# ishine/zerovox.cpp

Measured on AMD Instinct MI355X. Metric: audio-seconds/wall-second (xRT) end-to-end phoneme->22.05 kHz wav, higher is better.
Workload: dtype f16*f16->f32 (MFMA) convs, f32 (MFMA) attention/linear, f32 activations

## Files before the change

zerovox.cpp_amd/csrc/conv1d_mfma.hip:

```cpp
#include "kernels.h"
#include "knobs.h"
#include "mfma_common.h"
#include "tile_deal.h"

#include <hip/hip_fp16.h>
#include <algorithm>
#include <cstdlib>
#include <cstring>

namespace zv
{

#ifndef ZV_ST_AUX
#define ZV_ST_AUX 2
#endif
#ifdef ZV_ABL_A
#define ZV_ABL_LD(arr, p, mt) ((mt) == 0 ? *(const half8 *)(p) : arr[0])
#else
#define ZV_ABL_LD(arr, p, mt) (*(const half8 *)((p) + (mt) * 32 * RS))
#endif
#ifndef ZV_STAGE_U128
#define ZV_STAGE_U128 12
#endif
#ifndef ZV_STAGE_U256
// ... 94 lines not shown

void pack_pair_weight(const uint16_t *w, int K, int C, int Cp, uint16_t *dst)
{
    const int nkc = Cp / 16;
    const size_t seg = (size_t)(round_up(K * nkc, 4) + 8) * 512;
    memset(dst, 0, pair_weight_halfs(Cp, K) * 2);
    for (int nt = 0; nt < Cp / 32; nt++)
        for (int tap = 0; tap < K; tap++)
            for (int kc = 0; kc < nkc; kc++)
            {
                uint16_t *d = dst + nt * seg + (size_t)(tap * nkc + kc) * 512;
                for (int lane = 0; lane < 64; lane++)
                    for (int j = 0; j < 8; j++)
                    {
                        const int oc = nt * 32 + (lane & 31), ic = kc * 16 + 8 * (lane >> 5) + j;
                        d[lane * 8 + j] = (oc < C && ic < C) ? w[((size_t)oc * C + ic) * K + tap] : (uint16_t)0;
                    }
            }
}

__device__ __forceinline__ float lrelu_max(float x, float s)
{
    float r;
    const float xs = x * s;
    asm("v_max_f32 %0, %1, %2" : "=v"(r) : "v"(x), "v"(xs));
    return r;
}

__device__ __forceinline__ float lrelu_max_pre(float x, float xs)
{
    float r;
    asm("v_max_f32 %0, %1, %2" : "=v"(r) : "v"(x), "v"(xs));
    return r;
}

typedef unsigned int u32x4 __attribute__((ext_vector_type(4)));

typedef _Float16 half2v __attribute__((ext_vector_type(2)));

__device__ __forceinline__ uint2 lrelu4_f16(float x0, float x1, float x2, float x3, float sl)
{
    const float2v a = {x0, x1}, c = {x2, x3};
    const float2v as = a * sl, cs = c * sl;
    const float2v ra = {lrelu_max_pre(a[0], as[0]), lrelu_max_pre(a[1], as[1])};
    const float2v rc = {lrelu_max_pre(c[0], cs[0]), lrelu_max_pre(c[1], cs[1])};
    const half2v ha = __builtin_convertvector(ra, half2v), hc = __builtin_convertvector(rc, half2v);
    uint2 pk;
    pk.x = *(const unsigned int *)&ha;
    pk.y = *(const unsigned int *)&hc;
    return pk;
}


template <int U, int CP>
__device__ __forceinline__ void stage_act_buf(__amdgpu_buffer_rsrc_t rsrc, char *smem, int row_t0, int rows, int tid, float slope)
{
    constexpr int RS = CP * 2 + 16, COLS = CP / 4, SH = (CP == 32) ? 3 : (CP == 64 ? 4 : (CP == 128 ? 5 : 6));
    const int total = rows * COLS;
    for (int base = tid; base < total; base += 256 * U)
    {
        u32x4 v[U];
#pragma unroll
        for (int u = 0; u < U; u++)
        {
            const int idx = base + u * 256;
            const int r = idx >> SH, c4 = idx & (COLS - 1);
            const int voff = (idx < total) ? ((row_t0 + r) * CP + c4 * 4) * 4 : -16;
            v[u] = __builtin_amdgcn_raw_buffer_load_b128(rsrc, voff, 0, 0);
        }
#pragma unroll
        for (int u = 0; u < U; u++)
        {
            const int idx = base + u * 256;
            if (idx < total)
            {
                const int r = idx >> SH, c4 = idx & (COLS - 1);
                half4 h;
                h[0] = (_Float16)lrelu_max(__uint_as_float(v[u].x), slope);
                h[1] = (_Float16)lrelu_max(__uint_as_float(v[u].y), slope);
                h[2] = (_Float16)lrelu_max(__uint_as_float(v[u].z), slope);
                h[3] = (_Float16)lrelu_max(__uint_as_float(v[u].w), slope);
                *(half4 *)(smem + r * RS + c4 * 8) = h;
            }
        }
    }
}


size_t pair_weight16_halfs(int Cp, int K) { return pair_weight_halfs(Cp, K); }

void pack_pair_weight16(const uint16_t *w, int K, int C, int Cp, uint16_t *dst, bool conv2_layout)
{
    const int nk2 = Cp / 32;
    const size_t seg = (size_t)(round_up(K * (Cp / 16), 4) + 8) * 512;
    memset(dst, 0, pair_weight16_halfs(Cp, K) * 2);
    for (int nt = 0; nt < Cp / 32; nt++)
        for (int tap = 0; tap < K; tap++)
            for (int k2 = 0; k2 < nk2; k2++)
                for (int wt = 0; wt < 2; wt++)
                {
                    uint16_t *d = dst + nt * seg + ((size_t)(tap * nk2 + k2) * 2 + wt) * 512;
                    for (int lane = 0; lane < 64; lane++)
                        for (int j = 0; j < 8; j++)
                        {
                            const int r = lane & 15, g = lane >> 4;
                            const int oc = nt * 32 + (conv2_layout ? 2 * r + wt : 16 * wt + r), ic = k2 * 32 + 8 * g + j;
                            d[lane * 8 + j] = (oc < C && ic < C) ? w[((size_t)oc * C + ic) * K + tap] : (uint16_t)0;
                        }
                }
}

template <int MT, int NT, bool SWAP, bool ZERO = false>
__device__ __forceinline__ void mfma16_step(floatx4 (&acc)[MT][NT][2][2], const half8 (&l)[MT][2], const half8 (&w)[NT][2])
{
    const floatx4 z = {0.f, 0.f, 0.f, 0.f};
#pragma unroll
    for (int mt = 0; mt < MT; mt++)
#pragma unroll
        for (int nt = 0; nt < NT; nt++)
#pragma unroll
            for (int wt = 0; wt < 2; wt++)
#pragma unroll
                for (int lt = 0; lt < 2; lt++)
                {
                    if constexpr (SWAP)
                        acc[mt][nt][wt][lt] = __builtin_amdgcn_mfma_f32_16x16x32_f16(w[nt][wt], l[mt][lt], ZERO ? z : acc[mt][nt][wt][lt], 0, 0, 0);
                    else
                        acc[mt][nt][wt][lt] = __builtin_amdgcn_mfma_f32_16x16x32_f16(l[mt][lt], w[nt][wt], ZERO ? z : acc[mt][nt][wt][lt], 0, 0, 0);
                }
}

template <int NT>
__device__ __forceinline__ void deep16_preload_b(half8 (&b0)[2][NT][2], const half8 *wq, size_t wseg)
{
#pragma unroll
    for (int u = 0; u < 2; u++)
#pragma unroll
        for (int nt = 0; nt < NT; nt++)
#pragma unroll
            for (int wt = 0; wt < 2; wt++) b0[u][nt][wt] = wq[nt * wseg + (u * 2 + wt) * 64];
}

template <int CP, int MT, int NT, bool SWAP>
__device__ __forceinline__ void mfma16_taps_deep(floatx4 (&acc)[MT][NT][2][2], const char *ap, int dilRS, const half8 *wq, size_t wseg, int K,
                                                 half8 (&b0)[2][NT][2])
{
    constexpr int RS = CP * 2 + 16, NK2 = CP / 32;
    constexpr int TPB = (NK2 >= 4) ? 1 : 4 / NK2;
    constexpr bool HALF = NK2 == 8;
    const int nsb = (K * NK2 + 1) >> 1;
    const int nb = nsb >> 1;
    half8 b1[2][NT][2];
    wq += 4 * 64;
    half8 a[4][MT][2];
#define ZV16_UN(un) ((un) >= 4 ? (un) - 4 : 0)
#define ZV16_A_ADDR(un) ((un) >= 4 ? tbn[(ZV16_UN(un) / NK2) % 4] + (ZV16_UN(un) % NK2) * 64 : tb[((un) / NK2) % 4] + ((un) % NK2) * 64)
#define ZV16_LOAD_A(un)                                                                                          \
    {                                                                                                            \
        const char *np_ = ZV16_A_ADDR(un);                                                                       \
        _Pragma("unroll") for (int mt = 0; mt < MT; mt++)                                                        \
            _Pragma("unroll") for (int lt = 0; lt < 2; lt++) a[(un) % 4][mt][lt] = *(const half8 *)(np_ + (mt * 32 + lt) * RS); \
    }
#define ZV16_STEP(u, bset) ZV16_LOAD_A((u) + 1) mfma16_step<MT, NT, SWAP>(acc, a[(u) % 4], bset[(u) % 2]); __builtin_amdgcn_sched_barrier(0);
#define ZV16_STEPZ(u, bset) ZV16_LOAD_A((u) + 1) mfma16_step<MT, NT, SWAP, true>(acc, a[(u) % 4], bset[(u) % 2]); __builtin_amdgcn_sched_barrier(0);
#define ZV16_BODY(FIRSTSTEP)                                                                                     \
    {                                                                                                            \
// ... 211 lines not shown
}
#endif

size_t pair_ring_weight_halfs(int Cp, int K) { return (size_t)K * (Cp / 16) * (Cp / 32) * 512; }

void pack_pair_weight_ring(const uint16_t *w, int K, int C, int Cp, uint16_t *dst, bool conv2_layout)
{
    const int nk2 = Cp / 32, nnt = Cp / 32;
    for (int tap = 0; tap < K; tap++)
        for (int k2 = 0; k2 < nk2; k2++)
            for (int nt = 0; nt < nnt; nt++)
                for (int wt = 0; wt < 2; wt++)
                {
                    uint16_t *d = dst + ((((size_t)(tap * nk2 + k2) * nnt + nt) * 2) + wt) * 512;
                    for (int lane = 0; lane < 64; lane++)
                        for (int j = 0; j < 8; j++)
                        {
                            const int r = lane & 15, g = lane >> 4;
                            const int oc = nt * 32 + (conv2_layout ? 2 * r + wt : 16 * wt + r), ic = k2 * 32 + 8 * g + j;
                            d[lane * 8 + j] = (oc < C && ic < C) ? w[((size_t)oc * C + ic) * K + tap] : (uint16_t)0;
                        }
                }
}

template <bool MERGE>
__global__ __launch_bounds__(256, 2) void resblock_pair64_kernel(const PairJobs jobs)
{
    constexpr int CP = 64, MT = 2, NT = 2, BM = 256, RS = CP * 2 + 16;
    constexpr int CHUNK = 8 * 1024;
    const int jz = (int)blockIdx.z, bx = (int)blockIdx.x;
    const int TM = BM - (MERGE ? jobs.kmax - 1 : jobs.j[jz].K - 1);
    const int tps = (jobs.segs.max_rows * jobs.rate + TM - 1) / TM;
    const int vt = tile_deal(bx, tps, jobs.segs.nseg, jobs.deal_c);
    if (vt >= tps * jobs.segs.nseg) return;
    const int useg = vt / tps;
    const Seg sg = seg_at(jobs.segs, useg);
    const int L = sg.rows * jobs.rate;
    const int t0 = (vt - useg * tps) * TM;
    if (t0 >= L) return;

#ifdef ZV_STAMPS
    const int stamp_wg = (int)(blockIdx.x + gridDim.x * blockIdx.z);
    if (jobs.stamp && threadIdx.x == 0 && stamp_wg < ZV_STAMP_WGS)
    {
        jobs.stamp[(size_t)stamp_wg * ZV_STAMP_N + 8] = __builtin_amdgcn_s_getreg(63492);
        jobs.stamp[(size_t)stamp_wg * ZV_STAMP_N + 9] = __builtin_amdgcn_s_getreg(63508);
    }
#endif
    ZV_STAMP(0)
    extern __shared__ __attribute__((aligned(1024))) char smem[];
    char *ring = smem + jobs.ring_off;
    const int tid = threadIdx.x;
    const int lane = tid & 63;
    const int wave = __builtin_amdgcn_readfirstlane(tid >> 6);
    const int lc = lane & 15, lg = lane >> 4;
    const char *abase = smem + (wave * 32 * MT + 2 * lc) * RS + lg * 16;
    const char *bl = ring + lane * 16;

    floatx4 msum[MERGE ? MT : 1][MERGE ? NT : 1][2][2];
    for (int jb = MERGE ? 0 : jz; jb < (MERGE ? jobs.njobs : jz + 1); jb++)
    {
        const PairJob &P = jobs.j[jb];
        const int K = P.K, dil = P.dil;
        const int h2 = (K - 1) / 2, h1 = h2 * dil;
        const float *y_seg = P.y + (size_t)sg.row0 * jobs.rate * CP;
        float *out_seg = (MERGE ? jobs.merge_out : P.out) + (size_t)sg.row0 * jobs.rate * CP;
        const int nchunk = 2 * K;
        const uint64_t w1a = (uint64_t)P.w1r + wave * 2048, w2a = (uint64_t)P.w2r + wave * 2048 - (uint64_t)K * CHUNK;
        const uint32_t w1lo = __builtin_amdgcn_readfirstlane((uint32_t)w1a), w1hi = __builtin_amdgcn_readfirstlane((uint32_t)(w1a >> 32));
        const uint32_t w2lo = __builtin_amdgcn_readfirstlane((uint32_t)w2a), w2hi = __builtin_amdgcn_readfirstlane((uint32_t)(w2a >> 32));
        auto issue = [&](int g) {
            const uint64_t base = g < K ? ((uint64_t)w1hi << 32 | w1lo) : ((uint64_t)w2hi << 32 | w2lo);
            const char *src = (const char *)base + (size_t)g * CHUNK + lane * 16;
            char *dst = ring + (g & 3) * CHUNK + wave * 2048;
            __builtin_amdgcn_global_load_lds((const __attribute__((address_space(1))) void *)src, (__attribute__((address_space(3))) void *)dst, 16, 0, 0);
            __builtin_amdgcn_global_load_lds((const __attribute__((address_space(1))) void *)(src + 1024), (__attribute__((address_space(3))) void *)(dst + 1024), 16, 0, 0);
        };
        if (MERGE && jb) __syncthreads();
        issue(0);
        issue(1);
        issue(2);

        const __amdgpu_buffer_rsrc_t rs_y = __builtin_amdgcn_make_buffer_rsrc((void *)y_seg, 0, L * CP * 4, 0x00020000);
        stage_act_buf<20, CP>(rs_y, smem, t0 - h2 - h1, BM + 2 * h1 + dil, tid, P.slope);
        const int nrows = (L - t0 < TM) ? (L - t0) : TM;
        const __amdgpu_buffer_rsrc_t rs_res = __builtin_amdgcn_make_buffer_rsrc((void *)(y_seg + (size_t)t0 * CP), 0, nrows * CP * 4, 0x00020000);
        const int voff0 = ((wave * 32 * MT + 8 * lg) * CP + 2 * lc) * 4;
        typedef unsigned int u32x2 __attribute__((ext_vector_type(2)));
        u32x2 resv[MT][NT][2][4];
        auto load_res = [&]() {
#pragma unroll
            for (int nt = 0; nt < NT; nt++)
#pragma unroll
                for (int mt = 0; mt < MT; mt++)
#pragma unroll
                    for (int lt = 0; lt < 2; lt++)
#pragma unroll
                        for (int i = 0; i < 4; i++)
                            resv[mt][nt][lt][i] = __builtin_amdgcn_raw_buffer_load_b64(rs_res, voff0 + nt * 128, (mt * 32 + 2 * i + lt) * CP * 4, 0);
        };
        if constexpr (!MERGE) load_res();
        ZV_STAMP(1)
        __syncthreads();
        ZV_STAMP(2)

        floatx4 acc[MT][NT][2][2];
        half8 a[2][MT][2], b[2][NT][2];
        int g = 0;
#define ZV_LDR(slot, aptr, boff)                                                                                      \
    {                                                                                                                 \
        const char *ap_ = (aptr);                                                                                     \
        _Pragma("unroll") for (int mt = 0; mt < MT; mt++)                                                             \
            _Pragma("unroll") for (int lt = 0; lt < 2; lt++) a[slot][mt][lt] = *(const half8 *)(ap_ + (mt * 32 + lt) * RS);    \
        _Pragma("unroll") for (int nt = 0; nt < NT; nt++)                                                             \
            _Pragma("unroll") for (int wt = 0; wt < 2; wt++) b[slot][nt][wt] = *(const half8 *)(bp_ + (boff) + (nt * 2 + wt) * 1024); \
    }
#define ZV_MF(slot, SW, Z)                                \
    mfma16_step<MT, NT, SW, Z>(acc, a[slot], b[slot]);    \
    __builtin_amdgcn_sched_barrier(0);
#define ZV_TAP(SW, Z0, tapstride)                                                                         \
    {                                                                                                     \
        const char *bp_ = bl + (g & 3) * CHUNK, *bn_ = bl + ((g + 1) & 3) * CHUNK;                        \
        ZV_LDR(1, ap + 64, 4 * 1024) ZV_MF(0, SW, Z0)                                                     \
        if (g + 2 < nchunk) asm volatile("s_waitcnt vmcnt(2)" ::: "memory");                              \
        else asm volatile("s_waitcnt vmcnt(0)" ::: "memory");                                             \
        __builtin_amdgcn_s_barrier();                                                                     \
        if (g + 3 < nchunk) issue(g + 3);                                                                 \
        __builtin_amdgcn_sched_barrier(0);                                                                \
        ap += (tapstride);                                                                                \
        bp_ = bn_;                                                                                        \
        ZV_LDR(0, ap, 0) ZV_MF(1, SW, false)                                                              \
        g++;                                                                                              \
    }
        {
            const char *ap = abase;
            {
                const char *bp_ = bl;
                ZV_LDR(0, ap, 0)
            }
            ZV_TAP(true, true, dil * RS)
            for (int tap = 1; tap < K; tap++) ZV_TAP(true, false, dil * RS)
        }
        ZV_STAMP(3)
        asm volatile("s_waitcnt lgkmcnt(0)" ::: "memory");
        __builtin_amdgcn_s_barrier();

        ZV_STAMP(4)
        {
            const float sl = P.slope;
            const bool edge = t0 - h2 < 0 || t0 - h2 + BM > L;
#pragma unroll
            for (int nt = 0; nt < NT; nt++)
            {
                float4 bq[2];
#pragma unroll
                for (int wt = 0; wt < 2; wt++) bq[wt] = *(const float4 *)(P.b1 + nt * 32 + 16 * wt + 4 * lg);
#pragma unroll
                for (int mt = 0; mt < MT; mt++)
#pragma unroll
                    for (int lt = 0; lt < 2; lt++)
                    {
                        const int i = wave * 32 * MT + mt * 32 + 2 * lc + lt;
                        const int t = t0 - h2 + i;
                        const bool in = !edge || (t >= 0 && t < L);
#pragma unroll
                        for (int wt = 0; wt < 2; wt++)
                        {
                            uint2 pk = lrelu4_f16(acc[mt][nt][wt][lt][0] + bq[wt].x, acc[mt][nt][wt][lt][1] + bq[wt].y,
                                                  acc[mt][nt][wt][lt][2] + bq[wt].z, acc[mt][nt][wt][lt][3] + bq[wt].w, sl);
                            if (edge)
                            {
                                pk.x = in ? pk.x : 0u;
                                pk.y = in ? pk.y : 0u;
                            }
                            *(uint2 *)(smem + i * RS + (nt * 32 + 16 * wt + 4 * lg) * 2) = pk;
                        }
                    }
            }
        }
        asm volatile("s_waitcnt lgkmcnt(0)" ::: "memory");
        __builtin_amdgcn_s_barrier();

        ZV_STAMP(5)
        {
            const char *ap = abase;
            {
                const char *bp_ = bl + (g & 3) * CHUNK;
                ZV_LDR(0, ap, 0)
            }
            ZV_TAP(false, true, RS)
            for (int tap = 1; tap < K; tap++) ZV_TAP(false, false, RS)
        }
#undef ZV_TAP
#undef ZV_MF
#undef ZV_LDR

        ZV_STAMP(6)
        if constexpr (MERGE) load_res();
        const __amdgpu_buffer_rsrc_t rs_out = __builtin_amdgcn_make_buffer_rsrc((void *)(out_seg + (size_t)t0 * CP), 0, nrows * CP * 4, 0x00020000);
#pragma unroll
        for (int nt = 0; nt < NT; nt++)
        {
            const float2 bias = *(const float2 *)(P.b2 + nt * 32 + 2 * lc);
            const int voff = voff0 + nt * 128;
#pragma unroll
            for (int mt = 0; mt < MT; mt++)
#pragma unroll
                for (int lt = 0; lt < 2; lt++)
#pragma unroll
                    for (int i = 0; i < 4; i++)
                    {
                        float v0 = (acc[mt][nt][0][lt][i] + bias.x) + __uint_as_float(resv[mt][nt][lt][i][0]);
                        float v1 = (acc[mt][nt][1][lt][i] + bias.y) + __uint_as_float(resv[mt][nt][lt][i][1]);
                        if constexpr (MERGE)
                        {
                            msum[mt][nt][0][lt][i] = jb == 0 ? v0 : msum[mt][nt][0][lt][i] + v0;
                            msum[mt][nt][1][lt][i] = jb == 0 ? v1 : msum[mt][nt][1][lt][i] + v1;
                            if (jb != jobs.njobs - 1) continue;
                            v0 = msum[mt][nt][0][lt][i];
                            v1 = msum[mt][nt][1][lt][i];
                        }
                        const u32x2 o = {__float_as_uint(v0), __float_as_uint(v1)};
                        __builtin_amdgcn_raw_buffer_store_b64(o, rs_out, voff, (mt * 32 + 2 * i + lt) * CP * 4, ZV_ST_AUX);
                    }
        }
#ifdef ZV_STAMPS
        asm volatile("s_waitcnt vmcnt(0)" ::: "memory");
#endif
        ZV_STAMP(7)
    }
}

__global__ __launch_bounds__(256, 2) void resblock_block64_kernel(const TripleJobs jobs)
{
    constexpr int CP = 64, MT = 2, NT = 2, BM = 256, RS = CP * 2 + 16;
    constexpr int CHUNK = 8 * 1024;
    const TripleJob &P = jobs.j[blockIdx.z];
    const int K = P.K, nd = P.n_dil;
    const int h2 = (K - 1) / 2;
    int sumd = 0, dmax = 1;
    for (int d = 0; d < nd; d++) { sumd += P.dil[d]; dmax = P.dil[d] > dmax ? P.dil[d] : dmax; }
    const int H = h2 * (sumd + nd);
    const int TM = BM - 2 * H;
    const int tps = (jobs.segs.max_rows * jobs.rate + TM - 1) / TM;
    const int vt = tile_deal((int)blockIdx.x, tps, jobs.segs.nseg, jobs.deal_c);
    if (vt >= tps * jobs.segs.nseg) return;
    const int useg = vt / tps;
    const Seg sg = seg_at(jobs.segs, useg);
    const int L = sg.rows * jobs.rate;
    const int t0 = (vt - useg * tps) * TM;
    if (t0 >= L) return;
    const float *y_seg = P.y + (size_t)sg.row0 * jobs.rate * CP;
    float *out_seg = P.out + (size_t)sg.row0 * jobs.rate * CP;
    const int XM = h2 * dmax;
    const int xrows = BM + 2 * XM + 2 * dmax;
    const bool edge = t0 - H < 0 || t0 - H + BM > L;

    extern __shared__ __attribute__((aligned(1024))) char smem[];
    char *ring = smem + jobs.ring_off;
    const int tid = threadIdx.x;
    const int lane = tid & 63;
    const int wave = __builtin_amdgcn_readfirstlane(tid >> 6);
    const int lc = lane & 15, lg = lane >> 4;
    const char *abase = smem + (wave * 32 * MT + 2 * lc) * RS + lg * 16;
    const char *bl = ring + lane * 16;
    const int nchunk = 2 * K * nd;
    uint32_t wlo[2 * TRIPLE_MAX_DIL], whi[2 * TRIPLE_MAX_DIL];
#pragma unroll
    for (int c = 0; c < 2 * TRIPLE_MAX_DIL; c++)
    {
        const int d = c >> 1 < nd ? c >> 1 : 0;
        const uint64_t a = (uint64_t)((c & 1) ? P.w2[d] : P.w1[d]) + wave * 2048;
        wlo[c] = __builtin_amdgcn_readfirstlane((uint32_t)a);
        whi[c] = __builtin_amdgcn_readfirstlane((uint32_t)(a >> 32));
    }
    auto issue = [&](int g) {
        const int c = g / K, tap = g - c * K;
        uint32_t lo = wlo[0], hi = whi[0];
#pragma unroll
        for (int q = 1; q < 2 * TRIPLE_MAX_DIL; q++)
            if (c == q) { lo = wlo[q]; hi = whi[q]; }
        const char *src = (const char *)((uint64_t)hi << 32 | lo) + (size_t)tap * CHUNK + lane * 16;
        char *dst = ring + (g & 3) * CHUNK + wave * 2048;
        __builtin_amdgcn_global_load_lds((const __attribute__((address_space(1))) void *)src, (__attribute__((address_space(3))) void *)dst, 16, 0, 0);
        __builtin_amdgcn_global_load_lds((const __attribute__((address_space(1))) void *)(src + 1024), (__attribute__((address_space(3))) void *)(dst + 1024), 16, 0, 0);
    };
    issue(0);
    issue(1);
    issue(2);
    for (int i = tid; i < xrows * RS / 16; i += 256) ((uint4 *)smem)[i] = make_uint4(0, 0, 0, 0);
    typedef unsigned int u32x2 __attribute__((ext_vector_type(2)));
    float yreg[MT][NT][2][2][4];
    {
        const __amdgpu_buffer_rsrc_t rs_y = __builtin_amdgcn_make_buffer_rsrc((void *)y_seg, 0, L * CP * 4, 0x00020000);
        const int voff = ((t0 - H + wave * 32 * MT + 8 * lg) * CP + 2 * lc) * 4;
#pragma unroll
        for (int nt = 0; nt < NT; nt++)
#pragma unroll
            for (int mt = 0; mt < MT; mt++)
#pragma unroll
                for (int lt = 0; lt < 2; lt++)
#pragma unroll
                    for (int i = 0; i < 4; i++)
                    {
                        const u32x2 v = __builtin_amdgcn_raw_buffer_load_b64(rs_y, voff + nt * 128 + (mt * 32 + 2 * i + lt) * CP * 4, 0, 0);
                        yreg[mt][nt][0][lt][i] = __uint_as_float(v[0]);
                        yreg[mt][nt][1][lt][i] = __uint_as_float(v[1]);
                    }
    }
    __syncthreads();
    const float sl = P.slope;
    int g = 0;
    floatx4 acc[MT][NT][2][2];
    half8 a[2][MT][2], b[2][NT][2];
#define ZV_LDR(slot, aptr, boff)                                                                                      \
    {                                                                                                                 \
        const char *ap_ = (aptr);                                                                                     \
        _Pragma("unroll") for (int mt = 0; mt < MT; mt++)                                                             \
            _Pragma("unroll") for (int lt = 0; lt < 2; lt++) a[slot][mt][lt] = *(const half8 *)(ap_ + (mt * 32 + lt) * RS);    \
        _Pragma("unroll") for (int nt = 0; nt < NT; nt++)                                                             \
            _Pragma("unroll") for (int wt = 0; wt < 2; wt++) b[slot][nt][wt] = *(const half8 *)(bp_ + (boff) + (nt * 2 + wt) * 1024); \
    }
#define ZV_MF(slot, SW, Z)                                \
    mfma16_step<MT, NT, SW, Z>(acc, a[slot], b[slot]);    \
    __builtin_amdgcn_sched_barrier(0);
#define ZV_TAP(SW, Z0, tapstride)                                                                         \
    {                                                                                                     \
        const char *bp_ = bl + (g & 3) * CHUNK, *bn_ = bl + ((g + 1) & 3) * CHUNK;                        \
        ZV_LDR(1, ap + 64, 4 * 1024) ZV_MF(0, SW, Z0)                                                     \
        if (g + 2 < nchunk) asm volatile("s_waitcnt vmcnt(2)" ::: "memory");                              \
        else asm volatile("s_waitcnt vmcnt(0)" ::: "memory");                                             \
        __builtin_amdgcn_s_barrier();                                                                     \
        if (g + 3 < nchunk) issue(g + 3);                                                                 \
        __builtin_amdgcn_sched_barrier(0);                                                                \
        ap += (tapstride);                                                                                \
        bp_ = bn_;                                                                                        \
        ZV_LDR(0, ap, 0) ZV_MF(1, SW, false)                                                              \
        g++;                                                                                              \
    }
    for (int d = 0; d < nd; d++)
    {
        const int dil = P.dil[d], h1 = h2 * dil;
        {
#pragma unroll
            for (int nt = 0; nt < NT; nt++)
#pragma unroll
                for (int mt = 0; mt < MT; mt++)
#pragma unroll
                    for (int lt = 0; lt < 2; lt++)
#pragma unroll
                        for (int i = 0; i < 4; i++)
                        {
                            const int row = wave * 32 * MT + mt * 32 + 8 * lg + 2 * i + lt;
                            half2v h;
                            h[0] = (_Float16)lrelu_max(yreg[mt][nt][0][lt][i], sl);
                            h[1] = (_Float16)lrelu_max(yreg[mt][nt][1][lt][i], sl);
                            *(half2v *)(smem + (XM + row) * RS + (nt * 32 + 2 * lc) * 2) = h;
                        }
        }
        asm volatile("s_waitcnt lgkmcnt(0)" ::: "memory");
        __builtin_amdgcn_s_barrier();
        {
            const char *ap = abase + (XM - h1) * RS;
            {
                const char *bp_ = bl + (g & 3) * CHUNK;
                ZV_LDR(0, ap, 0)
            }
            ZV_TAP(true, true, dil * RS)
            for (int tap = 1; tap < K; tap++) ZV_TAP(true, false, dil * RS)
        }
        asm volatile("s_waitcnt lgkmcnt(0)" ::: "memory");
        __builtin_amdgcn_s_barrier();
        {
            const float *b1 = P.b1[d];
#pragma unroll
            for (int nt = 0; nt < NT; nt++)
            {
                float4 bq[2];
#pragma unroll
                for (int wt = 0; wt < 2; wt++) bq[wt] = *(const float4 *)(b1 + nt * 32 + 16 * wt + 4 * lg);
#pragma unroll
                for (int mt = 0; mt < MT; mt++)
#pragma unroll
                    for (int lt = 0; lt < 2; lt++)
                    {
                        const int i = wave * 32 * MT + mt * 32 + 2 * lc + lt;
                        const int t = t0 - H + i;
                        const bool in = !edge || (t >= 0 && t < L);
#pragma unroll
                        for (int wt = 0; wt < 2; wt++)
                        {
                            uint2 pk = lrelu4_f16(acc[mt][nt][wt][lt][0] + bq[wt].x, acc[mt][nt][wt][lt][1] + bq[wt].y,
                                                  acc[mt][nt][wt][lt][2] + bq[wt].z, acc[mt][nt][wt][lt][3] + bq[wt].w, sl);
                            if (edge)
                            {
                                pk.x = in ? pk.x : 0u;
                                pk.y = in ? pk.y : 0u;
                            }
                            *(uint2 *)(smem + (XM + i) * RS + (nt * 32 + 16 * wt + 4 * lg) * 2) = pk;
                        }
                    }
            }
        }
        asm volatile("s_waitcnt lgkmcnt(0)" ::: "memory");
        __builtin_amdgcn_s_barrier();
        {
            const char *ap = abase + (XM - h2) * RS;
            {
                const char *bp_ = bl + (g & 3) * CHUNK;
                ZV_LDR(0, ap, 0)
            }
            ZV_TAP(false, true, RS)
            for (int tap = 1; tap < K; tap++) ZV_TAP(false, false, RS)
        }
        {
            const float *b2 = P.b2[d];
#pragma unroll
            for (int nt = 0; nt < NT; nt++)
            {
                const float2 bias = *(const float2 *)(b2 + nt * 32 + 2 * lc);
#pragma unroll
                for (int mt = 0; mt < MT; mt++)
#pragma unroll
                    for (int lt = 0; lt < 2; lt++)
#pragma unroll
                        for (int i = 0; i < 4; i++)
                        {
                            const float v0 = (acc[mt][nt][0][lt][i] + bias.x) + yreg[mt][nt][0][lt][i];
                            const float v1 = (acc[mt][nt][1][lt][i] + bias.y) + yreg[mt][nt][1][lt][i];
                            bool in = true;
                            if (edge)
                            {
                                const int t = t0 - H + wave * 32 * MT + mt * 32 + 8 * lg + 2 * i + lt;
                                in = t >= 0 && t < L;
                            }
                            yreg[mt][nt][0][lt][i] = in ? v0 : 0.f;
                            yreg[mt][nt][1][lt][i] = in ? v1 : 0.f;
                        }
            }
        }
        if (d + 1 < nd)
        {
            asm volatile("s_waitcnt lgkmcnt(0)" ::: "memory");
            __builtin_amdgcn_s_barrier();
        }
    }
#undef ZV_TAP
#undef ZV_MF
#undef ZV_LDR
    const __amdgpu_buffer_rsrc_t rs_out = __builtin_amdgcn_make_buffer_rsrc((void *)out_seg, 0, L * CP * 4, 0x00020000);
#pragma unroll
    for (int nt = 0; nt < NT; nt++)
#pragma unroll
        for (int mt = 0; mt < MT; mt++)
#pragma unroll
            for (int lt = 0; lt < 2; lt++)
#pragma unroll
                for (int i = 0; i < 4; i++)
                {
                    const int row = wave * 32 * MT + mt * 32 + 8 * lg + 2 * i + lt;
                    const int t = t0 - H + row;
                    const int voff = (row >= H && row < H + TM && t >= 0) ? (t * CP + nt * 32 + 2 * lc) * 4 : -8;
                    const u32x2 o = {__float_as_uint(yreg[mt][nt][0][lt][i]), __float_as_uint(yreg[mt][nt][1][lt][i])};
                    __builtin_amdgcn_raw_buffer_store_b64(o, rs_out, voff, 0, ZV_ST_AUX);
                }
}

static inline BlockDesc block_desc(const TripleJob &P)
{
    BlockDesc b{P.Cp, P.K, P.n_dil, {0, 0, 0}};
    for (int d = 0; d < P.n_dil && d < TRIPLE_MAX_DIL; d++) b.dil[d] = P.dil[d];
    return b;
}

hipError_t launch_block64(hipStream_t s, const TripleJob *jobs, int njobs, const Segs &segs, int rate)
{
    if (njobs < 1 || njobs > PAIR_MAX_JOBS || segs.nseg < 1 || segs.max_rows < 1) return hipErrorInvalidValue;
    TripleJobs js;
    BlockDesc desc[PAIR_MAX_JOBS];
    for (int i = 0; i < njobs; i++)
    {
        js.j[i] = jobs[i];
        js.j[i].dbg = 0;
        desc[i] = block_desc(jobs[i]);
    }
    for (int i = njobs; i < PAIR_MAX_JOBS; i++) js.j[i] = js.j[0];
    const Block64Plan p = block64_plan(desc, ConvCall{njobs, segs.nseg, segs.max_rows, rate, 0, 0});
    if (!p.valid) return hipErrorInvalidValue;
    js.segs = segs;
    js.rate = rate;
    js.interleave = 1;
    js.db_mask = 0;
    js.deal_c = p.deal_c;
    js.ring_off = p.ring_off;
    return launch_lds(resblock_block64_kernel, dim3(p.gx, 1, p.gz), dim3(p.threads), p.lds_bytes, s, js);
}

template <int CP, int MT, bool MERGE>
static hipError_t launch_pair_cfg(hipStream_t s, const PairJobs &js, const PairPlan &p)
{
    size_t lds = p.lds_bytes;
#ifdef ZV_DIAG
    lds += (size_t)knob(ZV_LDS_PAD);
#endif
    return launch_lds(resblock_pair_kernel<CP, MT, MERGE>, dim3(p.gx, 1, p.gz), dim3(256), lds, s, js);
}

hipError_t launch_pair(hipStream_t s, const PairJob *jobs, int njobs, int n_cu, const Segs &segs, int rate, float *merge_out)
{
    if (njobs < 1 || njobs > PAIR_MAX_JOBS || segs.nseg < 1 || segs.max_rows < 1) return hipErrorInvalidValue;
    const int dbg = diag_bits();
    PairJobs js;
    js.segs = segs;
    js.rate = rate;
    js.njobs = njobs;
    js.merge_out = merge_out;
#ifdef ZV_STAMPS
    js.stamp = knob(ZV_STAMP_CP) && knob(ZV_STAMP_CP) == jobs[0].Cp && !merge_out ? stamp_buffer() : nullptr;
#endif
    int  Kmax = 0, dmax = 0;
    bool any_sum = false, all_ring = true;
    for (int i = 0; i < njobs; i++)
    {
        js.j[i] = jobs[i];
        js.j[i].dbg = dbg;
        if (jobs[i].Cp != jobs[0].Cp) return hipErrorInvalidValue;
        Kmax = jobs[i].K > Kmax ? jobs[i].K : Kmax;
        dmax = jobs[i].dil > dmax ? jobs[i].dil : dmax;
        any_sum = any_sum || jobs[i].sum_out || jobs[i].sum_in;
// ... 94 lines not shown
        if (!(ZV_DBGBITS(P.dbg) & 2))
            mfma_taps_deep<CP, MT, 1, true>(acc, abase + (XM - h1) * RS, dil * RS, (const half8 *)P.w1[d] + lane, wseg, K, bw);
        deep_preload_b<1>(bw, (const half8 *)P.w2[d] + lane, wseg);
        __syncthreads();
        {
            const int hh = lane >> 5;
            float4 bq[4];
#pragma unroll
            for (int q = 0; q < 4; q++) bq[q] = *(const float4 *)(P.b1[d] + 8 * q + 4 * hh);
#pragma unroll
            for (int mt = 0; mt < MT; mt++)
            {
                const int i = wave * 32 * MT + mt * 32 + (lane & 31);
                const int t = t0 - H + i;
                const bool in = !edge || (t >= 0 && t < L);
#pragma unroll
                for (int q = 0; q < 4; q++)
                {
                    half4 h;
                    h[0] = (_Float16)lrelu_max(acc[mt][0][4 * q + 0] + bq[q].x, sl);
                    h[1] = (_Float16)lrelu_max(acc[mt][0][4 * q + 1] + bq[q].y, sl);
                    h[2] = (_Float16)lrelu_max(acc[mt][0][4 * q + 2] + bq[q].z, sl);
                    h[3] = (_Float16)lrelu_max(acc[mt][0][4 * q + 3] + bq[q].w, sl);
                    uint2 pk = *(uint2 *)&h;
                    if (edge)
                    {
                        pk.x = in ? pk.x : 0u;
                        pk.y = in ? pk.y : 0u;
                    }
                    *(uint2 *)(smem + (XM + i) * RS + (8 * q + 4 * hh) * 2) = pk;
                }
            }
        }
        __syncthreads();

        if (!(ZV_DBGBITS(P.dbg) & 2))
            mfma_taps_deep<CP, MT, 1, false>(acc, abase + (XM - h2) * RS, RS, (const half8 *)P.w2[d] + lane, wseg, K, bw);
        if (d + 1 < nd) deep_preload_b<1>(bw, (const half8 *)P.w1[d + 1] + lane, wseg);
        {
            const float bias = P.b2[d][col];
            if (edge)
            {
#pragma unroll
                for (int mt = 0; mt < MT; mt++)
#pragma unroll
                    for (int r = 0; r < 16; r++)
                    {
                        const int t = t0 - H + irow0 + mt * 32 + (r & 3) + 8 * (r >> 2);
                        const float v = (acc[mt][0][r] + bias) + yreg[mt][r];
                        yreg[mt][r] = (t >= 0 && t < L) ? v : 0.f;
                    }
            }
            else
            {
#pragma unroll
                for (int mt = 0; mt < MT; mt++)
#pragma unroll
                    for (int r = 0; r < 16; r++) yreg[mt][r] = (acc[mt][0][r] + bias) + yreg[mt][r];
            }
        }
    }

    if (ZV_DBGBITS(P.dbg) & 4) return;
    const __amdgpu_buffer_rsrc_t rs_out = __builtin_amdgcn_make_buffer_rsrc((void *)out_seg, 0, L * CP * 4, 0x00020000);
#pragma unroll
    for (int mt = 0; mt < MT; mt++)
#pragma unroll
        for (int r = 0; r < 16; r++)
        {
            const int i = irow0 + mt * 32 + (r & 3) + 8 * (r >> 2);
            const int t = t0 - H + i;
            const int voff = (i >= H && i < H + TM && t >= 0) ? (t * CP + col) * 4 : -4;
            __builtin_amdgcn_raw_buffer_store_b32(__float_as_uint(yreg[mt][r]), rs_out, voff, 0, ZV_ST_AUX);
        }
}

__device__ __forceinline__ void dma_weights32(const void *wsrc, char *wlds, int nblk, int wave, int lane, int nwv)
{
    for (int blk = wave; blk < nblk; blk += nwv)
        __builtin_amdgcn_global_load_lds((const __attribute__((address_space(1))) void *)((const char *)wsrc + blk * 1024 + lane * 16),
                                         (__attribute__((address_space(3))) void *)(wlds + blk * 1024), 16, 0, 0);
}

template <int OFF>
__device__ __forceinline__ void lds_st_b64(unsigned addr, uint2 v)
{
    asm volatile("ds_write_b64 %0, %1 offset:%2" : : "v"(addr), "v"(v), "n"(OFF) : "memory");
}
template <int MT, bool SWAP>
__device__ __forceinline__ void mfma32x_ldsw(floatx4 (&acc)[MT][1][2][2], const char *ap, int dilRS, const char *wl, int K)
{
    constexpr int RS = 32 * 2 + 16;
    half8 a[2][MT][2], b[2][1][2];
#define ZV_LD(slot, aptr, woff)                                                                                       \
    {                                                                                                                 \
        const char *ap_ = (aptr);                                                                                     \
        _Pragma("unroll") for (int mt = 0; mt < MT; mt++)                                                             \
            _Pragma("unroll") for (int lt = 0; lt < 2; lt++) a[slot][mt][lt] = *(const half8 *)(ap_ + (mt * 32 + lt) * RS);    \
        _Pragma("unroll") for (int wt = 0; wt < 2; wt++) b[slot][0][wt] = *(const half8 *)(wl + (woff) + wt * 1024);   \
    }
#define ZV_ST(slot, Z)                                     \
    mfma16_step<MT, 1, SWAP, Z>(acc, a[slot], b[slot]);    \
    __builtin_amdgcn_sched_barrier(0);
    const char *t1 = ap + dilRS;
    ZV_LD(0, ap, 0)
    ZV_LD(1, t1, 2 * 1024) ZV_ST(0, true)
    for (int it = (K - 1) >> 1; it > 0; it--)
    {
        const char *t2 = t1 + dilRS, *t3 = t2 + dilRS;
        ZV_LD(0, t2, 4 * 1024) ZV_ST(1, false)
        ZV_LD(1, t3, 6 * 1024) ZV_ST(0, false)
        t1 = t3;
        wl += 4 * 1024;
    }
#undef ZV_ST
#undef ZV_LD
}

template <int OFF>
__device__ __forceinline__ void lds_st_b32(unsigned addr, unsigned v)
{
    asm volatile("ds_write_b32 %0, %1 offset:%2" : : "v"(addr), "v"(v), "n"(OFF) : "memory");
}
template <int MT_, int I = 0>
__device__ __forceinline__ void xwrite_all16(unsigned xa, const floatx4 (&y)[MT_][2][2], float sl)
{
    constexpr int mt = I / 2, lt = I % 2;
    const floatx4 s0 = y[mt][0][lt] * sl, s1 = y[mt][1][lt] * sl;
#define ZV_XW(i)                                                                                                  \
    {                                                                                                             \
        const float2v r = {lrelu_max_pre(y[mt][0][lt][i], s0[i]), lrelu_max_pre(y[mt][1][lt][i], s1[i])};      \
        const half2v h = __builtin_convertvector(r, half2v);                                                     \
        lds_st_b32<(mt * 32 + 2 * i + lt) * 80>(xa, *(const unsigned *)&h);                                       \
    }
    ZV_XW(0) ZV_XW(1) ZV_XW(2) ZV_XW(3)
#undef ZV_XW
    if constexpr (I + 1 < MT_ * 2) xwrite_all16<MT_, I + 1>(xa, y, sl);
}
template <int MT_, int I = 0>
__device__ __forceinline__ void pack_all16(unsigned pa, const uint2 (&pk)[MT_][2][2])
{
    constexpr int mt = I / 4, lt = (I / 2) % 2, wt = I % 2;
    lds_st_b64<(mt * 32 + lt) * 80 + 32 * wt>(pa, pk[mt][lt][wt]);
    if constexpr (I + 1 < MT_ * 4) pack_all16<MT_, I + 1>(pa, pk);
}

template <int MT, int R>
__global__ __launch_bounds__(64 * (R / 32 / MT), (MT >= 4 ? 2 : 4)) void resblock_block32_kernel(const TripleJobs jobs)
{
    constexpr int CP = 32, NWV = R / 32 / MT, NTH = 64 * NWV;
    constexpr int RS = CP * 2 + 16, NKC = CP / 16;
    const int il = jobs.interleave;
    const int bx = il > 1 ? (int)(((blockIdx.x >> 3) / il) << 3 | (blockIdx.x & 7)) : (int)blockIdx.x;
    const int jb = il > 1 ? (int)((blockIdx.x >> 3) % il) : (int)blockIdx.z;
    const TripleJob &P = jobs.j[jb];
    int H;
    {
        int sumd0 = 0;
        for (int d = 0; d < P.n_dil; d++) sumd0 += P.dil[d];
        H = ((P.K - 1) / 2) * (sumd0 + P.n_dil);
    }
    const int TM = R - 2 * H;
    const int tps = (jobs.segs.max_rows * jobs.rate + TM - 1) / TM;
    const int vt = tile_deal(bx, tps, jobs.segs.nseg, jobs.deal_c);
    if (vt >= tps * jobs.segs.nseg) return;
    const int useg = vt / tps;
    const Seg sg = seg_at(jobs.segs, useg);
    const int L = sg.rows * jobs.rate;
    const int t0 = (vt - useg * tps) * TM;
    if (t0 >= L) return;
    const bool edge = t0 - H < 0 || t0 - H + R > L;
// ... 229 lines not shown
```

Baseline: 33380.

## Overlap residual loads with activation staging and reorder block64 prologue loads

Adds a branch-free activation staging variant that clamps out-of-range indices and writes LDS via inline ds_write_b64. The post-staging __syncthreads becomes a partial vmcnt wait plus s_barrier, so residual buffer loads stay in flight across the barrier. In the block64 resblock kernel, the y register loads are issued before the LDS zero-fill and weight ring requests, and the weight base pointers move to scalar locals passed to a helper. The aim is to hide global-load latency in the prologue, at the cost of relying on exact vmcnt ordering, which is fragile if the load count changes.

```diff
diff --git a/zerovox.cpp_amd/csrc/conv1d_mfma.hip b/zerovox.cpp_amd/csrc/conv1d_mfma.hip
--- a/zerovox.cpp_amd/csrc/conv1d_mfma.hip
+++ b/zerovox.cpp_amd/csrc/conv1d_mfma.hip
@@ -200,6 +200,43 @@
                 h[3] = (_Float16)lrelu_max(__uint_as_float(v[u].w), slope);
                 *(half4 *)(smem + r * RS + c4 * 8) = h;
             }
+        }
+    }
+}
+
+template <int OFF>
+__device__ __forceinline__ void lds_st_b64(unsigned addr, uint2 v)
+{
+    asm volatile("ds_write_b64 %0, %1 offset:%2" : : "v"(addr), "v"(v), "n"(OFF) : "memory");
+}
+
+template <int U, int CP>
+__device__ __forceinline__ void stage_act_buf_flat(__amdgpu_buffer_rsrc_t rsrc, char *smem, int row_t0, int rows, int tid, float slope)
+{
+    constexpr int RS = CP * 2 + 16, COLS = CP / 4, SH = (CP == 32) ? 3 : (CP == 64 ? 4 : (CP == 128 ? 5 : 6));
+    const int total = rows * COLS;
+    for (int base = tid; base < total; base += 256 * U)
+    {
+        u32x4 v[U];
+#pragma unroll
+        for (int u = 0; u < U; u++)
+        {
+            const int idx = (base + u * 256 < total) ? base + u * 256 : base;
+            const int r = idx >> SH, c4 = idx & (COLS - 1);
+            v[u] = __builtin_amdgcn_raw_buffer_load_b128(rsrc, ((row_t0 + r) * CP + c4 * 4) * 4, 0, 0);
+        }
+        __builtin_amdgcn_sched_barrier(0);
+#pragma unroll
+        for (int u = 0; u < U; u++)
+        {
+            const int idx = (base + u * 256 < total) ? base + u * 256 : base;
+            const int r = idx >> SH, c4 = idx & (COLS - 1);
+            half4 h;
+            h[0] = (_Float16)lrelu_max(__uint_as_float(v[u].x), slope);
+            h[1] = (_Float16)lrelu_max(__uint_as_float(v[u].y), slope);
+            h[2] = (_Float16)lrelu_max(__uint_as_float(v[u].z), slope);
+            h[3] = (_Float16)lrelu_max(__uint_as_float(v[u].w), slope);
+            lds_st_b64<0>((unsigned)(uintptr_t)(smem + r * RS + c4 * 8), *(const uint2 *)&h);
         }
     }
 }
@@ -577,7 +614,7 @@
         issue(2);
 
         const __amdgpu_buffer_rsrc_t rs_y = __builtin_amdgcn_make_buffer_rsrc((void *)y_seg, 0, L * CP * 4, 0x00020000);
-        stage_act_buf<20, CP>(rs_y, smem, t0 - h2 - h1, BM + 2 * h1 + dil, tid, P.slope);
+        stage_act_buf_flat<20, CP>(rs_y, smem, t0 - h2 - h1, BM + 2 * h1 + dil, tid, P.slope);
         const int nrows = (L - t0 < TM) ? (L - t0) : TM;
         const __amdgpu_buffer_rsrc_t rs_res = __builtin_amdgcn_make_buffer_rsrc((void *)(y_seg + (size_t)t0 * CP), 0, nrows * CP * 4, 0x00020000);
         const int voff0 = ((wave * 32 * MT + 8 * lg) * CP + 2 * lc) * 4;
@@ -596,7 +633,10 @@
         };
         if constexpr (!MERGE) load_res();
         ZV_STAMP(1)
-        __syncthreads();
+        constexpr int RES_LOADS = MERGE ? 0 : MT * NT * 2 * 4;
+        static_assert(RES_LOADS < 64, "s_waitcnt vmcnt is a 6-bit count");
+        asm volatile("s_waitcnt vmcnt(%0) lgkmcnt(0)" ::"n"(RES_LOADS) : "memory");
+        __builtin_amdgcn_s_barrier();
         ZV_STAMP(2)
 
         floatx4 acc[MT][NT][2][2];
@@ -724,6 +764,23 @@
 #endif
         ZV_STAMP(7)
     }
+}
+
+__device__ __forceinline__ void ring_request64(int g, int K, uint32_t lo0, uint32_t hi0, uint32_t lo1, uint32_t hi1, uint32_t lo2, uint32_t hi2,
+                                               uint32_t lo3, uint32_t hi3, uint32_t lo4, uint32_t hi4, uint32_t lo5, uint32_t hi5, char *ring, int wave,
+                                               int lane)
+{
+    const int c = g / K, tap = g - c * K;
+    uint32_t lo = lo0, hi = hi0;
+    if (c == 1) { lo = lo1; hi = hi1; }
+    if (c == 2) { lo = lo2; hi = hi2; }
+    if (c == 3) { lo = lo3; hi = hi3; }
+    if (c == 4) { lo = lo4; hi = hi4; }
+    if (c == 5) { lo = lo5; hi = hi5; }
+    const char *src = (const char *)((uint64_t)hi << 32 | lo) + (size_t)tap * (8 * 1024) + lane * 16;
+    char *dst = ring + (g & 3) * (8 * 1024) + wave * 2048;
+    __builtin_amdgcn_global_load_lds((const __attribute__((address_space(1))) void *)src, (__attribute__((address_space(3))) void *)dst, 16, 0, 0);
+    __builtin_amdgcn_global_load_lds((const __attribute__((address_space(1))) void *)(src + 1024), (__attribute__((address_space(3))) void *)(dst + 1024), 16, 0, 0);
 }
 
 __global__ __launch_bounds__(256, 2) void resblock_block64_kernel(const TripleJobs jobs)
@@ -760,32 +817,8 @@
     const char *abase = smem + (wave * 32 * MT + 2 * lc) * RS + lg * 16;
     const char *bl = ring + lane * 16;
     const int nchunk = 2 * K * nd;
-    uint32_t wlo[2 * TRIPLE_MAX_DIL], whi[2 * TRIPLE_MAX_DIL];
-#pragma unroll
-    for (int c = 0; c < 2 * TRIPLE_MAX_DIL; c++)
-    {
-        const int d = c >> 1 < nd ? c >> 1 : 0;
-        const uint64_t a = (uint64_t)((c & 1) ? P.w2[d] : P.w1[d]) + wave * 2048;
-        wlo[c] = __builtin_amdgcn_readfirstlane((uint32_t)a);
-        whi[c] = __builtin_amdgcn_readfirstlane((uint32_t)(a >> 32));
-    }
-    auto issue = [&](int g) {
-        const int c = g / K, tap = g - c * K;
-        uint32_t lo = wlo[0], hi = whi[0];
-#pragma unroll
-        for (int q = 1; q < 2 * TRIPLE_MAX_DIL; q++)
-            if (c == q) { lo = wlo[q]; hi = whi[q]; }
-        const char *src = (const char *)((uint64_t)hi << 32 | lo) + (size_t)tap * CHUNK + lane * 16;
-        char *dst = ring + (g & 3) * CHUNK + wave * 2048;
-        __builtin_amdgcn_global_load_lds((const __attribute__((address_space(1))) void *)src, (__attribute__((address_space(3))) void *)dst, 16, 0, 0);
-        __builtin_amdgcn_global_load_lds((const __attribute__((address_space(1))) void *)(src + 1024), (__attribute__((address_space(3))) void *)(dst + 1024), 16, 0, 0);
-    };
-    issue(0);
-    issue(1);
-    issue(2);
-    for (int i = tid; i < xrows * RS / 16; i += 256) ((uint4 *)smem)[i] = make_uint4(0, 0, 0, 0);
     typedef unsigned int u32x2 __attribute__((ext_vector_type(2)));
-    float yreg[MT][NT][2][2][4];
+    u32x2 yraw[MT][NT][2][4];
     {
         const __amdgpu_buffer_rsrc_t rs_y = __builtin_amdgcn_make_buffer_rsrc((void *)y_seg, 0, L * CP * 4, 0x00020000);
         const int voff = ((t0 - H + wave * 32 * MT + 8 * lg) * CP + 2 * lc) * 4;
@@ -797,13 +830,36 @@
                 for (int lt = 0; lt < 2; lt++)
 #pragma unroll
                     for (int i = 0; i < 4; i++)
-                    {
-                        const u32x2 v = __builtin_amdgcn_raw_buffer_load_b64(rs_y, voff + nt * 128 + (mt * 32 + 2 * i + lt) * CP * 4, 0, 0);
-                        yreg[mt][nt][0][lt][i] = __uint_as_float(v[0]);
-                        yreg[mt][nt][1][lt][i] = __uint_as_float(v[1]);
-                    }
-    }
+                        yraw[mt][nt][lt][i] = __builtin_amdgcn_raw_buffer_load_b64(rs_y, voff + nt * 128 + (mt * 32 + 2 * i + lt) * CP * 4, 0, 0);
+    }
+    __builtin_amdgcn_sched_barrier(0);
+    for (int i = tid; i < xrows * RS / 16; i += 256) ((uint4 *)smem)[i] = make_uint4(0, 0, 0, 0);
+    __builtin_amdgcn_sched_barrier(0);
+    static_assert(TRIPLE_MAX_DIL == 3, "six conv base pointers");
+#define ZV_WBASE(c)                                                                                                   \
+    const uint64_t wa##c = (uint64_t)(((c) & 1) ? P.w2[((c) >> 1) < nd ? ((c) >> 1) : 0] : P.w1[((c) >> 1) < nd ? ((c) >> 1) : 0]) + wave * 2048; \
+    const uint32_t wlo##c = __builtin_amdgcn_readfirstlane((uint32_t)wa##c), whi##c = __builtin_amdgcn_readfirstlane((uint32_t)(wa##c >> 32));
+    ZV_WBASE(0) ZV_WBASE(1) ZV_WBASE(2) ZV_WBASE(3) ZV_WBASE(4) ZV_WBASE(5)
+#undef ZV_WBASE
+#define ZV_ISSUE(g) ring_request64((g), K, wlo0, whi0, wlo1, whi1, wlo2, whi2, wlo3, whi3, wlo4, whi4, wlo5, whi5, ring, wave, lane)
+    ZV_ISSUE(0);
+    ZV_ISSUE(1);
+    ZV_ISSUE(2);
     __syncthreads();
+    float yreg[MT][NT][2][2][4];
+#pragma unroll
+    for (int nt = 0; nt < NT; nt++)
+#pragma unroll
+        for (int mt = 0; mt < MT; mt++)
+#pragma unroll
+            for (int lt = 0; lt < 2; lt++)
+#pragma unroll
+                for (int i = 0; i < 4; i++)
+                {
+                    asm volatile("" : "+v"(yraw[mt][nt][lt][i]));
+                    yreg[mt][nt][0][lt][i] = __uint_as_float(yraw[mt][nt][lt][i][0]);
+                    yreg[mt][nt][1][lt][i] = __uint_as_float(yraw[mt][nt][lt][i][1]);
+                }
     const float sl = P.slope;
     int g = 0;
     floatx4 acc[MT][NT][2][2];
@@ -826,7 +882,7 @@
         if (g + 2 < nchunk) asm volatile("s_waitcnt vmcnt(2)" ::: "memory");                              \
         else asm volatile("s_waitcnt vmcnt(0)" ::: "memory");                                             \
         __builtin_amdgcn_s_barrier();                                                                     \
-        if (g + 3 < nchunk) issue(g + 3);                                                                 \
+        if (g + 3 < nchunk) ZV_ISSUE(g + 3);                                                              \
         __builtin_amdgcn_sched_barrier(0);                                                                \
         ap += (tapstride);                                                                                \
         bp_ = bn_;                                                                                        \
@@ -940,6 +996,7 @@
             __builtin_amdgcn_s_barrier();
         }
     }
+#undef ZV_ISSUE
 #undef ZV_TAP
 #undef ZV_MF
 #undef ZV_LDR
@@ -1200,11 +1257,6 @@
                                          (__attribute__((address_space(3))) void *)(wlds + blk * 1024), 16, 0, 0);
 }
 
-template <int OFF>
-__device__ __forceinline__ void lds_st_b64(unsigned addr, uint2 v)
-{
-    asm volatile("ds_write_b64 %0, %1 offset:%2" : : "v"(addr), "v"(v), "n"(OFF) : "memory");
-}
 template <int MT, bool SWAP>
 __device__ __forceinline__ void mfma32x_ldsw(floatx4 (&acc)[MT][1][2][2], const char *ap, int dilRS, const char *wl, int K)
 {
```

Result: no change. 33500 (median of 6 runs) (+0.4%).
